# nitishsaDire/objectDetection_ssd

Measured on AMD Instinct MI355X. Metric: images/sec SSD300-VGG16 train step, higher is better.
Workload: dtype f32 (tensors, accumulators, loss, SGD; the Winograd-domain products of the layers with >= 256 reduction channels are formed from three EXACT bf16 limbs per f32 operand on the bf16 MFMA -- six limb products per f32 product, dropped terms <= 2^-26 -- measured no further from f64 than the f32 MFMA; SSD

## Files before the change

### include/ssd_gfx950.h

```cpp
#ifndef SSD_GFX950_H
#define SSD_GFX950_H

#include <stddef.h>
#include <stdint.h>

#ifdef __cplusplus
extern "C" {
#endif

#define SSD_ABI_VERSION 1

enum ssd_status {
    SSD_OK = 0,
    SSD_ERR_BAD_SHAPE = -1,
    SSD_ERR_WORKSPACE = -2,
    SSD_ERR_NULL = -3,
    SSD_ERR_LAUNCH = -4,
    SSD_ERR_ALIGN = -5
};

int ssd_abi_version(void);
const char* ssd_status_string(int status);

typedef struct ssd_conv_geom {
// ... 105 lines not shown
int ssd_wino4_dy_transform_pooled(const float* dpool, const unsigned char* argmax, const float* y_pooled, int Hp, int Wp, int ldy,
                                  const ssd_conv_geom* g, float* wgrad_planes, float* dgrad_planes_out, float* bias_partial, void* stream);
int ssd_conv3x3_wino_wgrad_planes_pooled(const float* planes, const float* dpool, const unsigned char* argmax, const float* y_pooled,
                                         int Hp, int Wp, int ldy, float* dw_oihw, float* dbias, const ssd_conv_geom* g,
                                         float* dgrad_planes_out, void* workspace, size_t workspace_bytes, void* stream);
int ssd_conv3x3_wino_fwd_keep_bits(const float* x, const float* U_fwd, const float* bias, float* y, int ldy, const ssd_conv_geom* g, int relu,
                                   float* planes_keep, uint64_t* relu_bits_out, void* workspace, size_t workspace_bytes, void* stream);
int ssd_conv3x3_wino_fwd_pool_bits(const float* x, const float* U_fwd, const float* bias, float* y_pooled, uint8_t* argmax,
                                   const ssd_conv_geom* g, int ceil_mode, float* planes_keep, uint64_t* relu_bits_out, void* workspace,
                                   size_t workspace_bytes, void* stream);
int ssd_conv3x3_wino_dgrad_bits(const float* dy, int ldy, const float* U_bwd, int Co_pad, float* dx, const uint64_t* relu_bits, int accumulate,
                                const ssd_conv_geom* g, void* workspace, size_t workspace_bytes, void* stream);
int ssd_conv3x3_wino_dgrad_planes_bits(const float* dy_planes, const float* U_bwd, int Co_pad, float* dx, const uint64_t* relu_bits,
                                       int accumulate, const ssd_conv_geom* g, void* workspace, size_t workspace_bytes, void* stream);
int ssd_conv3x3_wino_wgrad_planes(const float* planes, const float* dy, int ldy, float* dw_oihw, float* dbias, const ssd_conv_geom* g,
                                  float* dgrad_planes_out, void* workspace, size_t workspace_bytes, void* stream);
int ssd_conv3x3_wino_dgrad_planes(const float* dy_planes, const float* U_bwd, int Co_pad, float* dx, const float* relu_mask,
                                  int accumulate, const ssd_conv_geom* g, void* workspace, size_t workspace_bytes, void* stream);
int ssd_conv1_first_wino_fwd(const float* x_nchw, const float* w_rows, const float* bias, float* planes, uint64_t* relu_bits, int N, int H, int W,
                             void* stream);
int ssd_conv3x3_wino_fwd_from_planes(const float* planes, const float* U_fwd, const float* bias, float* y, int ldy, float* y_pooled, uint8_t* argmax,
                                     const ssd_conv_geom* g, int relu, int ceil_mode, void* workspace, size_t workspace_bytes, void* stream);
int ssd_wino_weights_adj(const float* w_oihw, float* U_adj, int Co, int Ci, int Co_pad, void* stream);
size_t ssd_wino4_adj_planes_floats(const ssd_conv_geom* g);
int ssd_conv3x3_wino_dgrad_adj_gemm(const float* y_planes, int ldy, const float* U_adj, float* md_planes, const ssd_conv_geom* g, void* stream);
int ssd_wino4_adj_output(const float* md_planes, float* dx, const float* relu_mask, const uint64_t* relu_bits, int accumulate,
                         const ssd_conv_geom* g, void* stream);
int ssd_wino4_adj_output_to_planes(const float* md_planes, const float* relu_mask, const uint64_t* relu_bits, const ssd_conv_geom* g,
                                   const ssd_conv_geom* g_below, float* y_planes, float* bias_partial, void* stream);
int ssd_tune_set_wino_bias_tail(int on);
int ssd_tune_set_wino_xform_blocks(int blocks);
int ssd_tune_set_wino_fused(int mode);
int ssd_gemm_planes_x3v2(const void* a3, const void* w3, float* out, int M, int K, int N, int n_rows, int nbatch, int dither, void* stream);
int ssd_tune_set_x3_big(int mode);
int ssd_tune_set_x3_mfma(int rows);
int ssd_tune_set_gemm_nt(int mode);
int ssd_wino_uses_x3(int mo, int K);
int ssd_tune_set_wino_x3(int on);
size_t ssd_gemm_x3_weights_bytes(int rows, int K, int nbatch);
int ssd_gemm_x3_split_weights(const float* w, void* w3, int rows, int K, int nbatch, void* stream);
int ssd_gemm_planes_x3(const float* a, const void* w3, float* out, int M, int K, int N, int n_rows, int nbatch, void* stream);
int ssd_conv1x1_fwd_x3(const float* x, const void* w3, const float* bias, float* y, int ldy, const ssd_conv_geom* g, int relu, void* stream);
int ssd_conv1x1_dgrad_x3(const float* dy, int ldy, const void* w3t, float* dx, const float* relu_mask, int accumulate, const ssd_conv_geom* g,
                         void* stream);
size_t ssd_conv1x1_wgrad_x3_workspace(const ssd_conv_geom* g, int ldy);
int ssd_conv1x1_wgrad_x3(const float* x, const float* dy, int ldy, float* dw, float* dbias, const ssd_conv_geom* g, void* workspace,
                         size_t workspace_bytes, void* stream);
int ssd_gemm_planes_f32(const float* a, const float* w, float* out, int M, int K, int N, int n_rows, int nbatch, void* stream);
int ssd_has_experimental(void);
int ssd_tune_set_wino_full(int mode);
int ssd_conv3x3_wino_uses_full(const ssd_conv_geom* g, int direction);
int ssd_tune_set_wino_fused_stagger(int cycles);
int ssd_tune_set_wino_fused_stamps(uint64_t* device_buffer);
int ssd_tune_set_wino_wgrad_tn(int on);
int ssd_prof_gemm_begin(void);
int ssd_prof_gemm_collect_kinds(float* ms_out, double* flops_out, int* kinds_out, int max);
int ssd_prof_gemm_collect(float* ms_out, double* flops_out, int max);
int ssd_tune_set_igemm(int tile, int nbuf);
int ssd_tune_set_igemm_stamps(uint64_t* device_buffer);
int ssd_tune_set_dgrad_parity(int on);
int ssd_tune_set_batched_units(int on);
int ssd_tune_set_igemm_lds_pad(int bytes);
int ssd_tune_set_wgrad(int bt, int nbuf, int blocks_per_cu);
int ssd_tune_set_wgrad_patch(int shape);

int ssd_im2col_first(const float* x_nchw, float* out, int N, int H, int W, void* stream);
int ssd_conv1_first_fwd(const float* x_nchw, const float* w_rows, const float* bias, float* y_nhwc, float* col_out, int N, int H, int W,
                        int relu, void* stream);
size_t ssd_conv1_first_wgrad_workspace(int N, int H, int W);
int ssd_conv1_first_wgrad(const float* x_nchw, const float* dy_nhwc, float* dw_rows, float* dbias, int N, int H, int W, void* workspace,
                          size_t workspace_bytes, void* stream);

int ssd_im2col_nchw3(const float* x_nchw, float* out, int N, int H, int W, int R, int S, int stride, int pad,
                     int Ho, int Wo, int Kpad, void* stream);
int ssd_conv2d_fwd_accum(const float* x, const float* w_ohwi, const float* bias, float* y_inout, int ldy,
                         const ssd_conv_geom* g, int relu, void* stream);
int ssd_conv2d_fwd_accum_bf16(const float* x, const float* w_ohwi, const float* bias, float* y_inout, int ldy,
                              const ssd_conv_geom* g, int relu, void* stream);
int ssd_channel_affine(const float* x, const float* scale, const float* shift, float* y, size_t M, int C, int relu,
                       void* stream);

int ssd_maxpool_fwd(const float* x, float* y, uint8_t* argmax, int N, int H, int W, int C,
                    int k, int stride, int pad, int Ho, int Wo, void* stream);
int ssd_maxpool_bwd(const float* dy, const uint8_t* argmax, float* dx, const float* relu_mask, int accumulate,
                    int N, int H, int W, int C, int k, int stride, int pad, int Ho, int Wo, void* stream);
int ssd_maxpool_bwd_gated(const float* dy, const uint8_t* argmax, const float* y, float* dx, int N, int H, int W, int C,
                          int k, int stride, int pad, int Ho, int Wo, void* stream);

int ssd_l2norm_fwd(const float* x, const float* gamma, float* y, int M, int C, void* stream);
size_t ssd_l2norm_bwd_workspace(int M, int C);
int ssd_l2norm_bwd(const float* x, const float* gamma, const float* dy, float* dx, float* dgamma,
                   int M, int C, void* workspace, size_t workspace_bytes, void* stream);

int ssd_heads_scatter(const float* packed, int ld, float* loc, float* conf, int N, int HW, int A,
                      int prior_off, int P, int n_classes, void* stream);
int ssd_heads_gather(const float* dloc, const float* dconf, float* packed, int ld, int N, int HW, int A,
                     int prior_off, int P, int n_classes, void* stream);

int ssd_tune_set_loss_form(int three_launch);
size_t ssd_multibox_loss_workspace(int bs, int P, int n_gt);
int ssd_multibox_loss(const float* loc, const float* conf, const float* gt_boxes, const float* gt_classes,
                      const int32_t* img_start, int bs, int n_gt, const float* priors_cxcywh,
                      const float* priors_xyxy, int P, int n_classes, float iou_threshold, int neg_pos_ratio,
                      int norm_mode, float* losses, int32_t* obj, int32_t* cls, float* dloc, float* dconf,
                      void* workspace, size_t workspace_bytes, void* stream);

// ... 80 lines not shown
```

### objectdetection_ssd_amd/_lib.py

```python
from __future__ import annotations

import ctypes as C
import os

PKG = os.path.dirname(os.path.abspath(__file__))
LIB_PATH = os.path.join(PKG, "libssd_gfx950.so")

SSD_ABI_VERSION = 1


class ConvGeom(C.Structure):
    _fields_ = [(n, C.c_int32) for n in ("N", "H", "W", "Ci", "Ho", "Wo", "Co", "R", "S", "stride", "pad", "dil")]


class ImageDesc(C.Structure):
    _fields_ = [("src_offset", C.c_int64)] + [(n, C.c_int32) for n in (
        "src_h", "src_w", "canvas_h", "canvas_w", "place_top", "place_left", "crop_top", "crop_left", "crop_h", "crop_w",
        "flip", "reserved")]


class WeightJob(C.Structure):
    _fields_ = [("w0", C.c_void_p), ("w1", C.c_void_p), ("out_fwd", C.c_void_p), ("out_bwd", C.c_void_p)] + [(n, C.c_int32) for n in (
        "co0", "co", "ci", "taps", "co_pad", "kind", "pad0", "pad1")]

# ... 76 lines not shown
    "ssd_conv3x3_halo_fwd_bf16": (_I, [_P, _P, _I, _P, _P, _I, _G, _I, _P]),
    "ssd_conv3x3_halo_dgrad_bf16": (_I, [_P, _I, _P, _I, _P, _P, _I, _G, _P]),
    "ssd_conv2d_wgrad_workspace": (_Z, [_G]),
    "ssd_conv2d_wgrad": (_I, [_P, _P, _I, _P, _P, _G, _P, _Z, _P]),
    "ssd_conv2d_igemm_tile": (_I, [_G, _I, C.POINTER(C.c_int), C.POINTER(C.c_int)]),
    "ssd_conv2d_wgrad_tile": (_I, [_G, C.POINTER(C.c_int), C.POINTER(C.c_int)]),
    "ssd_conv2d_wgrad_plan": (_I, [_G, _I, C.POINTER(C.c_int)]),
    "ssd_conv3x3_bf16_plan": (_I, [_I, _I, _I, _I, _I, C.POINTER(C.c_int)]),
    "ssd_conv3x3_halo_shape": (_I, [_G, _I, _I]),
    "ssd_conv2d_igemm_workspace": (_Z, [_G, _I]),
    "ssd_conv2d_fwd_ws": (_I, [_P, _P, _P, _P, _I, _G, _I, _P, _Z, _P]),
    "ssd_conv2d_dgrad_ws": (_I, [_P, _I, _P, _I, _P, _P, _I, _G, _P, _Z, _P]),
    "ssd_tune_set_igemm_splitk": (_I, [_I]),
    "ssd_wino_weights": (_I, [_P, _P, _P, _I, _I, _I, _I, _P]),
    "ssd_conv3x3_wino_workspace": (_Z, [_G, _I, _I]),
    "ssd_conv3x3_wino_fwd": (_I, [_P, _P, _P, _P, _I, _G, _I, _I, _P, _Z, _P]),
    "ssd_conv3x3_wino_fwd_pool": (_I, [_P, _P, _P, _P, _P, _G, _I, _P, _P, _Z, _P]),
    "ssd_conv3x3_wino_fwd_keep": (_I, [_P, _P, _P, _P, _I, _G, _I, _P, _P, _Z, _P]),
    "ssd_weight_job_blocks": (_I, [_P]),
    "ssd_weights_prepare": (_I, [_P, _P, _I, _I, _P]),
    "ssd_wino4_bias_partial_floats": (_Z, [_G, _I]),
    "ssd_wino4_dy_transform": (_I, [_P, _I, _G, _P, _P, _P, _P]),
    "ssd_wino_weights_adj": (_I, [_P, _P, _I, _I, _I, _P]),
    "ssd_conv1_first_wino_fwd": (_I, [_P, _P, _P, _P, _P, _I, _I, _I, _P]),
    "ssd_conv3x3_wino_fwd_from_planes": (_I, [_P, _P, _P, _P, _I, _P, _P, _G, _I, _I, _P, _Z, _P]),
    "ssd_wino4_adj_planes_floats": (_Z, [_G]),
    "ssd_conv3x3_wino_dgrad_adj_gemm": (_I, [_P, _I, _P, _P, _G, _P]),
    "ssd_wino4_adj_output": (_I, [_P, _P, _P, _P, _I, _G, _P]),
    "ssd_wino4_adj_output_to_planes": (_I, [_P, _P, _P, _G, _G, _P, _P, _P]),
    "ssd_wino4_dy_transform_pooled": (_I, [_P, _P, _P, _I, _I, _I, _G, _P, _P, _P, _P]),
    "ssd_conv3x3_wino_wgrad_planes_pooled": (_I, [_P, _P, _P, _P, _I, _I, _I, _P, _P, _G, _P, _P, _Z, _P]),
    "ssd_wino4_wgrad_gemm_workspace": (_Z, [_G, _I]),
    "ssd_wino4_wgrad_gemm": (_I, [_P, _P, _I, _P, _P, _P, _G, _P, _Z, _P]),
    "ssd_conv3x3_wino_fwd_keep_bits": (_I, [_P, _P, _P, _P, _I, _G, _I, _P, _P, _P, _Z, _P]),
    "ssd_conv3x3_wino_fwd_pool_bits": (_I, [_P, _P, _P, _P, _P, _G, _I, _P, _P, _P, _Z, _P]),
    "ssd_conv3x3_wino_dgrad_planes_bits": (_I, [_P, _P, _I, _P, _P, _I, _G, _P, _Z, _P]),
    "ssd_conv3x3_wino_wgrad_planes": (_I, [_P, _P, _I, _P, _P, _G, _P, _P, _Z, _P]),
    "ssd_conv3x3_wino_dgrad_planes": (_I, [_P, _P, _I, _P, _P, _I, _G, _P, _Z, _P]),
    "ssd_conv3x3_wino_dgrad": (_I, [_P, _I, _P, _I, _P, _P, _I, _G, _I, _P, _Z, _P]),
    "ssd_conv3x3_wino_wgrad_workspace": (_Z, [_G, _I, _I]),
    "ssd_conv3x3_wino_wgrad": (_I, [_P, _P, _I, _P, _P, _G, _I, _P, _Z, _P]),
    "ssd_tune_set_wino_wgrad_tn": (_I, [_I]),
    "ssd_tune_set_wino_fused": (_I, [_I]),
    "ssd_tune_set_gemm_nt": (_I, [_I]),
    "ssd_tune_set_wino_bias_tail": (_I, [_I]),
    "ssd_tune_set_batched_units": (_I, [_I]),
    "ssd_tune_set_dgrad_parity": (_I, [_I]),
    "ssd_tune_set_wino_full": (_I, [_I]),
    "ssd_conv3x3_wino_uses_full": (_I, [_G, _I]),
    "ssd_conv3x3_wino_dgrad_bits": (_I, [_P, _I, _P, _I, _P, _P, _I, _G, _P, _Z, _P]),
    "ssd_tune_set_wino_xform_blocks": (_I, [_I]),
    "ssd_tune_set_wino_fused_stamps": (_I, [_P]),
    "ssd_tune_set_wino_fused_stagger": (_I, [_I]),
    "ssd_prof_gemm_begin": (_I, []),
    "ssd_prof_gemm_collect": (_I, [_P, _P, _I]),
    "ssd_prof_gemm_collect_kinds": (_I, [_P, _P, _P, _I]),
    "ssd_tune_set_igemm": (_I, [_I, _I]),
    "ssd_tune_set_igemm_lds_pad": (_I, [_I]),
    "ssd_tune_set_igemm_stamps": (_I, [_P]),
    "ssd_tune_set_wgrad": (_I, [_I, _I, _I]),
    "ssd_tune_set_wgrad_patch": (_I, [_I]),
    "ssd_im2col_first": (_I, [_P, _P, _I, _I, _I, _P]),
    "ssd_conv1_first_fwd": (_I, [_P, _P, _P, _P, _P, _I, _I, _I, _I, _P]),
    "ssd_conv1_first_wgrad_workspace": (_Z, [_I, _I, _I]),
    "ssd_conv1_first_wgrad": (_I, [_P, _P, _P, _P, _I, _I, _I, _P, _Z, _P]),
    "ssd_maxpool_fwd": (_I, [_P, _P, _P, _I, _I, _I, _I, _I, _I, _I, _I, _I, _P]),
    "ssd_maxpool_bwd_gated": (_I, [_P, _P, _P, _P, _I, _I, _I, _I, _I, _I, _I, _I, _I, _P]),
    "ssd_maxpool_bwd": (_I, [_P, _P, _P, _P, _I, _I, _I, _I, _I, _I, _I, _I, _I, _I, _P]),
    "ssd_l2norm_fwd": (_I, [_P, _P, _P, _I, _I, _P]),
    "ssd_l2norm_bwd_workspace": (_Z, [_I, _I]),
    "ssd_l2norm_bwd": (_I, [_P, _P, _P, _P, _P, _I, _I, _P, _Z, _P]),
    "ssd_heads_scatter": (_I, [_P, _I, _P, _P, _I, _I, _I, _I, _I, _I, _P]),
    "ssd_heads_gather": (_I, [_P, _P, _P, _I, _I, _I, _I, _I, _I, _I, _P]),
    "ssd_multibox_loss_workspace": (_Z, [_I, _I, _I]),
    "ssd_multibox_loss": (_I, [_P, _P, _P, _P, _P, _I, _I, _P, _P, _I, _I, _F, _I, _I, _P, _P, _P, _P, _P, _P, _Z, _P]),
    "ssd_decode_nms_workspace": (_Z, [_I, _I]),
    "ssd_decode_nms": (_I, [_P, _P, _P, _I, _I, _F, _F, _I, _F, _F, _P, _P, _P, _P, _P, _P, _Z, _P]),
    "ssd_decode_nms_batch_workspace": (_Z, [_I, _I, _I]),
    "ssd_decode_nms_batch": (_I, [_P, _P, _P, _P, _I, _I, _I, _F, _F, _I, _P, _P, _P, _P, _P, _P, _Z, _P]),
    "ssd_sgd_momentum": (_I, [_P, _P, _P, _Z, _F, _F, _F, _P, _I, _P]),
    "ssd_bn_workspace": (_Z, [_Z, _I]),
    "ssd_bn_train_stats": (_I, [_P, _I, _Z, _I, _P, _P, _F, _F, _P, _P, _P, _P, _P, _P, _P, _P, _Z, _P]),
    "ssd_bn_apply": (_I, [_P, _I, _Z, _I, _P, _P, _P, _I, _P, _P, _I, _I, _F, _U64, _I, _I, _P, _I, _P]),
    "ssd_bn_train_bwd": (_I, [_P, _I, _P, _I, _Z, _I, _P, _P, _P, _I, _F, _U64, _I, _I, _I, _P, _P, _P, _I, _P, _I, _P, _Z, _P]),
    "ssd_dropout_mask": (_I, [_P, _Z, _F, _U64, _I, _P]),
}

_lib = None


def load() -> C.CDLL:
    global _lib
    if _lib is not None:
        return _lib
    import torch
    if not os.path.exists(LIB_PATH):
        from . import build as _build
        _build.build()
    try:
        lib = C.CDLL(LIB_PATH)
    except OSError as e:
        raise RuntimeError(f"cannot load {LIB_PATH}: {e}.  The gfx950 HIP extension is the only compute "
                           f"path of this package; build it with `python -m objectdetection_ssd_amd.build`.") from e
    for name, (res, args) in SIGNATURES.items():
        fn = getattr(lib, name)
        fn.restype = res
# ... 12 lines not shown
```

### objectdetection_ssd_amd/csrc/wino_fused.hip

```cpp
#include "common.h"

namespace {

__device__ constexpr float F4_AT[4][6] = {{1, 1, 1, 1, 1, 0}, {0, 1, -1, 2, -2, 0}, {0, 1, 1, 4, 4, 0}, {0, 1, -1, 8, -8, 1}};

struct FusedParams {
    const float* V;
    const float* U;
    size_t plane_v, plane_u;
    int tiles, K, Nrows, Nout;
    int groups, nblk_n;
    float* out; int ldo; int Cvalid;
    const float* bias; const float* mask; const unsigned long long* mask_bits; int relu, accumulate;
    int H, W, TH, TW;
    float* yp; uint8_t* am; int Ho, Wo;
    unsigned long long* stamps;
    int stagger;
};

constexpr int FG = 32, FN = 64, FK = 64;
#ifndef WF_NS
#define WF_NS 5
#define WF_PD 3
#endif
constexpr int NS = WF_NS, PD = WF_PD;
constexpr int STAGE_F = (FG + FN) * FK;
constexpr int LOADS = 3;
constexpr int YS_F = FG * 16 * FN;
constexpr int LDS_F = NS * STAGE_F > YS_F ? NS * STAGE_F : YS_F;
static_assert(NS - PD >= 2, "a slot is re-filled no earlier than two barriers after its last read");
static_assert(LDS_F * 4 <= 160 * 1024, "LDS");

typedef __attribute__((address_space(3))) void lds_void;

template <int N> __device__ __forceinline__ void wait_vmcnt() { asm volatile("s_waitcnt vmcnt(%0)" ::"n"(N) : "memory"); }

template <int KCN>
__global__ __launch_bounds__(512, 2) void wino4_gemm_out_kernel(const FusedParams p) {
    __shared__ __attribute__((aligned(16))) float lds[LDS_F];
    const int tid = threadIdx.x, lane = tid & 63;
    const int wave = __builtin_amdgcn_readfirstlane(tid >> 6);
    const int mb = wave >> 2, nbw = wave & 3;
    const int nblk = p.groups * p.nblk_n;
    const int lid = xcd_swizzle(blockIdx.x, nblk);
    const int grp = lid / p.nblk_n, nb = lid - grp * p.nblk_n;
    const int tile0 = grp * FG, n0 = nb * FN;
    constexpr int S = 36 * KCN;
    const bool stamp = p.stamps != nullptr && (blockIdx.x & 15) == 0 && tid == 0;
    unsigned long long ts[8] = {0, 0, 0, 0, 0, 0, 0, 0};
    if (stamp) ts[0] = __builtin_readcyclecounter();
    if (p.stagger > 0 && blockIdx.x < 256) {
        const long long want = (long long)((blockIdx.x >> 3) & 7) * p.stagger;
        const long long t0 = (long long)__builtin_readcyclecounter();
        while ((long long)__builtin_readcyclecounter() - t0 < want) __builtin_amdgcn_s_sleep(64);
    }

    const int lrow = lane >> 4, pc = lane & 15;
    unsigned src_off[LOADS];
    bool is_a[LOADS];
    int lds_off[LOADS];
#pragma unroll
    for (int i = 0; i < LOADS; ++i) {
        const int q = 3 * wave + i;
        is_a[i] = q < 8;
        const int row = is_a[i] ? 4 * q + lrow : 4 * (q - 8) + lrow;
        const int src_row = is_a[i] ? min(tile0 + row, p.tiles - 1) : min(n0 + row, p.Nrows - 1);
        src_off[i] = (unsigned)src_row * (unsigned)p.K + (unsigned)((pc ^ (row & 15)) * 4);
        lds_off[i] = q * 256;
    }
    auto issue = [&](int stage) {
        const int xi = stage / KCN, kc = stage % KCN, slot = stage % NS;
        const float* vsrc = p.V + (size_t)xi * p.plane_v + kc * FK;
        const float* usrc = p.U + (size_t)xi * p.plane_u + kc * FK;
        float* base = lds + slot * STAGE_F;
#pragma unroll
        for (int i = 0; i < LOADS; ++i)
            __builtin_amdgcn_global_load_lds((is_a[i] ? vsrc : usrc) + src_off[i], (lds_void*)(base + lds_off[i]), 16, 0, 0);
    };

    f32x4 acc[36];
#pragma unroll
    for (int xi = 0; xi < 36; ++xi) acc[xi] = f32x4{0.f, 0.f, 0.f, 0.f};

    const int r15 = lane & 15, kq = lane >> 4;
    const int a_rd = (mb * 16 + r15) * FK, b_rd = FG * FK + (nbw * 16 + r15) * FK;
    int sw[4];
#pragma unroll
    for (int j = 0; j < 4; ++j) sw[j] = ((4 * j + kq) ^ r15) * 4;

    struct Frag { f32x4 a[4], b[4]; };
    Frag F[2];
    auto load_frags = [&](Frag& f, int slot) {
        const float* st = lds + slot * STAGE_F;
#pragma unroll
        for (int j = 0; j < 4; ++j) {
            f.a[j] = *reinterpret_cast<const f32x4*>(st + a_rd + sw[j]);
            f.b[j] = *reinterpret_cast<const f32x4*>(st + b_rd + sw[j]);
        }
    };
    auto mma4 = [&](f32x4& c, const Frag& f, int j) {
#ifdef WF_NO_MFMA
        c += f.a[j] * f.b[j];
#else
#pragma unroll
        for (int e = 0; e < 4; ++e) c = __builtin_amdgcn_mfma_f32_16x16x4f32(f.a[j][e], f.b[j][e], c, 0, 0, 0);
#endif
    };

#pragma unroll
    for (int s = 0; s < PD; ++s)
        if (s < S) issue(s);
    wait_vmcnt<(PD < S ? PD - 1 : S - 1) * LOADS>();
    __builtin_amdgcn_s_barrier();
    asm volatile("" ::: "memory");
    load_frags(F[0], 0);
    if (stamp) ts[1] = __builtin_readcyclecounter();

#pragma clang loop unroll(full)
    for (int s = 0; s < S; ++s) {
        f32x4& c = acc[s / KCN];
        const Frag& cur = F[s & 1];
        Frag& nxt = F[(s & 1) ^ 1];
        mma4(c, cur, 0);
        __builtin_amdgcn_sched_barrier(0);
#ifndef WF_NO_LOAD
        if (s + PD < S) issue(s + PD);
#endif
        __builtin_amdgcn_sched_barrier(0);
        mma4(c, cur, 1);
        mma4(c, cur, 2);
        __builtin_amdgcn_sched_barrier(0);
        if (s + 1 < S) {
            const int issued = (s + PD + 1 < S ? s + PD + 1 : S);
            const int ahead = issued - s - 2;
            if (ahead >= 3) wait_vmcnt<3 * LOADS>();
            else if (ahead == 2) wait_vmcnt<2 * LOADS>();
            else if (ahead == 1) wait_vmcnt<LOADS>();
            else wait_vmcnt<0>();
            __builtin_amdgcn_s_barrier();
            asm volatile("" ::: "memory");
            load_frags(nxt, (s + 1) % NS);
        }
        __builtin_amdgcn_sched_barrier(0);
        mma4(c, cur, 3);
    }

    if (stamp) ts[2] = __builtin_readcyclecounter();
    float* ys = lds;
    const int C4 = p.Nout >> 2;
    __builtin_amdgcn_s_barrier();
#pragma unroll
    for (int r = 0; r < 4; ++r) {
        float t[4][6];
#pragma unroll
        for (int b = 0; b < 6; ++b) {
            const float m0 = acc[b][r], m1 = acc[6 + b][r], m2 = acc[12 + b][r], m3 = acc[18 + b][r], m4 = acc[24 + b][r], m5 = acc[30 + b][r];
            const float s1 = m1 + m2, d1 = m1 - m2, s2 = m3 + m4, d2 = m3 - m4;
            t[0][b] = m0 + s1 + s2;
            t[1][b] = d1 + 2.f * d2;
            t[2][b] = s1 + 4.f * s2;
            t[3][b] = d1 + 8.f * d2 + m5;
        }
        float* dst = ys + (size_t)((mb * 16 + 4 * kq + r) * 16) * FN + nbw * 16 + r15;
#pragma unroll
        for (int i = 0; i < 4; ++i) {
            const float s1 = t[i][1] + t[i][2], d1 = t[i][1] - t[i][2], s2 = t[i][3] + t[i][4], d2 = t[i][3] - t[i][4];
            dst[(i * 4 + 0) * FN] = t[i][0] + s1 + s2;
            dst[(i * 4 + 1) * FN] = d1 + 2.f * d2;
            dst[(i * 4 + 2) * FN] = s1 + 4.f * s2;
            dst[(i * 4 + 3) * FN] = d1 + 8.f * d2 + t[i][5];
        }
    }
    asm volatile("s_waitcnt lgkmcnt(0)" ::: "memory");
    __builtin_amdgcn_s_barrier();
    if (stamp) ts[3] = __builtin_readcyclecounter();
    {
        const int tl = tid >> 4, c4l = tid & 15;
        const int tile = tile0 + tl, c4 = (n0 >> 2) + c4l;
        if (tile < p.tiles && c4 < C4) {
            const int tw = tile % p.TW, th = (tile / p.TW) % p.TH, n = tile / (p.TW * p.TH);
            const float* src = ys + (size_t)(tl * 16) * FN + c4l * 4;
            f32x4 bv = {0.f, 0.f, 0.f, 0.f};
            if (p.bias != nullptr) {
#pragma unroll
                for (int e = 0; e < 4; ++e) bv[e] = c4 * 4 + e < p.Cvalid ? p.bias[c4 * 4 + e] : 0.f;
            }
            if (p.yp == nullptr) {
                const unsigned long long word = p.mask_bits != nullptr ? p.mask_bits[(size_t)tile * C4 + c4] : 0ull;
#pragma unroll
                for (int a = 0; a < 4; ++a) {
                    const int oh = 4 * th + a;
                    if (oh >= p.H) continue;
#pragma unroll
                    for (int b = 0; b < 4; ++b) {
                        const int ow = 4 * tw + b;
                        if (ow >= p.W) continue;
                        f32x4 v = *reinterpret_cast<const f32x4*>(src + (a * 4 + b) * FN) + bv;
                        const size_t idx = (((size_t)n * p.H + oh) * p.W + ow) * p.ldo + c4 * 4;
                        if (p.accumulate) v += *reinterpret_cast<const f32x4*>(p.out + idx);
                        if (p.relu) {
#pragma unroll
                            for (int e = 0; e < 4; ++e) v[e] = v[e] < 0.f ? 0.f : v[e];
                        }
                        if (p.mask_bits != nullptr) {
#pragma unroll
                            for (int e = 0; e < 4; ++e) v[e] = ((word >> ((a * 4 + b) * 4 + e)) & 1ull) ? v[e] : 0.f;
                        } else if (p.mask != nullptr) {
                            const f32x4 mk = *reinterpret_cast<const f32x4*>(p.mask + idx);
#pragma unroll
                            for (int e = 0; e < 4; ++e) v[e] = mk[e] > 0.f ? v[e] : 0.f;
                        }
                        *reinterpret_cast<f32x4*>(p.out + idx) = v;
                    }
                }
            } else {
#pragma unroll
                for (int pa = 0; pa < 2; ++pa) {
                    const int oh = 2 * th + pa;
                    if (oh >= p.Ho) continue;
#pragma unroll
                    for (int pb = 0; pb < 2; ++pb) {
                        const int ow = 2 * tw + pb;
                        if (ow >= p.Wo) continue;
                        f32x4 best = {-INFINITY, -INFINITY, -INFINITY, -INFINITY};
                        int bi[4] = {0, 0, 0, 0};
                        bool first = true;
#pragma unroll
                        for (int r = 0; r < 2; ++r) {
                            if (2 * oh + r >= p.H) continue;
#pragma unroll
                            for (int q = 0; q < 2; ++q) {
                                if (2 * ow + q >= p.W) continue;
                                f32x4 v = *reinterpret_cast<const f32x4*>(src + ((2 * pa + r) * 4 + 2 * pb + q) * FN) + bv;
#pragma unroll
                                for (int e = 0; e < 4; ++e) {
                                    v[e] = v[e] < 0.f ? 0.f : v[e];
                                    if (first || v[e] > best[e] || v[e] != v[e]) {
                                        best[e] = v[e];
                                        bi[e] = r * 2 + q;
                                    }
                                }
                                first = false;
                            }
                        }
                        const size_t o = (((size_t)n * p.Ho + oh) * p.Wo + ow) * C4 + c4;
                        *reinterpret_cast<f32x4*>(p.yp + o * 4) = best;
                        if (p.am != nullptr)
                            *reinterpret_cast<uint32_t*>(p.am + o * 4) =
                                (uint32_t)bi[0] | ((uint32_t)bi[1] << 8) | ((uint32_t)bi[2] << 16) | ((uint32_t)bi[3] << 24);
                    }
                }
            }
        }
    }
    if (stamp) {
        ts[4] = __builtin_readcyclecounter();
        asm volatile("s_waitcnt vmcnt(0)" ::: "memory");
        unsigned long long* o = p.stamps + (size_t)(blockIdx.x >> 4) * 8;
        for (int i = 0; i < 5; ++i) o[i] = ts[i];
        o[5] = __builtin_readcyclecounter();
    }
}

}
int ssd_internal_prof_open(double flops, int kind, hipStream_t st);
void ssd_internal_prof_close(int slot, hipStream_t st);
namespace {
unsigned long long* g_fused_stamps = nullptr;
int g_fused_stagger = -1;
}

extern "C" int ssd_tune_set_wino_fused_stagger(int cycles) {
    g_fused_stagger = cycles;
    return SSD_OK;
}
extern "C" int ssd_tune_set_wino_fused_stamps(uint64_t* device_buffer) {
    g_fused_stamps = reinterpret_cast<unsigned long long*>(device_buffer);
    return SSD_OK;
}

__attribute__((visibility("hidden"))) int ssd_internal_wino4_gemm_out(const float* V, const float* U, int tiles, int K, int Nrows, int Nout,
                                                                       float* out, int ldo, int Cvalid, const float* bias, const float* mask,
                                                                       const unsigned long long* mask_bits, int relu, int accumulate, int H, int W,
                                                                       int TH, int TW, float* yp, uint8_t* am, int Ho, int Wo, hipStream_t st) {
    if ((K != 64 && K != 128 && K != 256) || tiles <= 0 || Nout <= 0 || Nout % 4 != 0 || Nrows <= 0) return SSD_ERR_BAD_SHAPE;
    if ((size_t)tiles * K >= (1ull << 32) || (size_t)Nrows * K >= (1ull << 32)) return SSD_ERR_BAD_SHAPE;
    FusedParams p;
    p.V = V; p.U = U;
    p.plane_v = (size_t)tiles * K; p.plane_u = (size_t)Nrows * K;
    p.tiles = tiles; p.K = K; p.Nrows = Nrows; p.Nout = Nout;
    p.groups = ssd_cdiv(tiles, FG); p.nblk_n = ssd_cdiv(Nout, FN);
    p.out = out; p.ldo = ldo; p.Cvalid = Cvalid; p.bias = bias; p.mask = mask; p.mask_bits = mask_bits; p.relu = relu; p.accumulate = accumulate;
    p.H = H; p.W = W; p.TH = TH; p.TW = TW;
    p.yp = yp; p.am = am; p.Ho = Ho; p.Wo = Wo;
    p.stamps = g_fused_stamps;
    p.stagger = g_fused_stagger < 0 ? 0 : g_fused_stagger;
    const long long nblk = (long long)p.groups * p.nblk_n;
    if (nblk >= (1ll << 31)) return SSD_ERR_BAD_SHAPE;
    const int slot = ssd_internal_prof_open(2.0 * 36 * tiles * (double)K * (double)(p.nblk_n * FN), 1, st);
    switch (K / FK) {
        case 1: hipLaunchKernelGGL(wino4_gemm_out_kernel<1>, dim3((unsigned)nblk), dim3(512), 0, st, p); break;
        case 2: hipLaunchKernelGGL(wino4_gemm_out_kernel<2>, dim3((unsigned)nblk), dim3(512), 0, st, p); break;
        case 4: hipLaunchKernelGGL(wino4_gemm_out_kernel<4>, dim3((unsigned)nblk), dim3(512), 0, st, p); break;
        default: return SSD_ERR_BAD_SHAPE;
    }
    ssd_internal_prof_close(slot, st);
    SSD_CHECK_LAUNCH();
    return SSD_OK;
}

namespace {

__device__ constexpr float F4_BT[6][6] = {{4, 0, -5, 0, 1, 0}, {0, -4, -4, 1, 1, 0}, {0, 4, -4, -1, 1, 0},
                                          {0, -2, -1, 2, 1, 0}, {0, 2, -1, -2, 1, 0}, {0, 4, 0, -5, 0, 1}};

struct FullParams {
    const float* x;
    unsigned x_bytes;
    const float* U;
    size_t plane_u;
    int tiles, K, Nrows, Nout, groups, nblk_n;
    float* out; int ldo; int Cvalid;
    const float* bias; const float* mask; const unsigned long long* mask_bits; int relu, accumulate;
    int H, W, TH, TW;
    float* yp; uint8_t* am; int Ho, Wo;
    float* V_keep;
    unsigned long long* bits_out;
    unsigned long long* stamps;
};

#ifdef SSD_EXPERIMENTAL
constexpr int GT = 32;
constexpr int KH = 32;
constexpr int VS_F = 36 * GT * KH;
typedef float f32x2 __attribute__((ext_vector_type(2)));

template <int KP>
__global__ __launch_bounds__(512, 2) void wino4_full_kernel(const FullParams p) {
    __shared__ __attribute__((aligned(16))) float lds[VS_F];
    const int tid = threadIdx.x, lane = tid & 63;
    const int wave = __builtin_amdgcn_readfirstlane(tid >> 6);
    const int nbw = wave & 3, mb = wave >> 2;
    const int nblk = p.groups * p.nblk_n;
    const int lid = xcd_swizzle(blockIdx.x, nblk);
    const int grp = lid / p.nblk_n, nb = lid - grp * p.nblk_n;
    const int tile0 = grp * GT, n0 = nb * FN;
    const int r15 = lane & 15, kq = lane >> 4;
    const bool stamp = p.stamps != nullptr && (blockIdx.x & 15) == 0 && tid == 0;
    unsigned long long ts[8] = {0, 0, 0, 0, 0, 0, 0, 0};
    if (stamp) ts[0] = __builtin_readcyclecounter();

    f32x4 acc[36];
#pragma unroll
    for (int i = 0; i < 36; ++i) acc[i] = f32x4{0.f, 0.f, 0.f, 0.f};

    const int brow = min(n0 + nbw * 16 + r15, p.Nrows - 1);
// ... 263 lines not shown
```

Measured before the change: 1612.

## Make fused Winograd GEMM kernel persistent with grid capped at CU count

The fused Winograd GEMM+output-transform kernel now loops over work tiles with a grid-stride loop, and by default launches at most one block per CU instead of one block per tile. The epilogue also reads the whole 16-pixel tile out of LDS into registers and then hits a barrier before the global stores, so the next iteration can safely reuse the LDS. The aim is to cut block launch and prologue overhead and even out the tail. The risk is lower occupancy: launch bounds allow two blocks per CU but the grid caps at one per CU. Each block also loses the overlap between one tile's epilogue and the next tile's loads, and the extra barrier plus register pressure could hurt.

```diff
diff --git a/include/ssd_gfx950.h b/include/ssd_gfx950.h
--- a/include/ssd_gfx950.h
+++ b/include/ssd_gfx950.h
@@ -181,6 +181,8 @@
 int ssd_conv3x3_wino_uses_full(const ssd_conv_geom* g, int direction);
 int ssd_tune_set_wino_fused_stagger(int cycles);
 int ssd_tune_set_wino_fused_stamps(uint64_t* device_buffer);
+int ssd_tune_set_wino_fused_persistent(int mode);
+int ssd_tune_set_wino_fused_grid(int blocks);
 int ssd_tune_set_wino_wgrad_tn(int on);
 int ssd_prof_gemm_begin(void);
 int ssd_prof_gemm_collect_kinds(float* ms_out, double* flops_out, int* kinds_out, int max);
diff --git a/objectdetection_ssd_amd/_lib.py b/objectdetection_ssd_amd/_lib.py
--- a/objectdetection_ssd_amd/_lib.py
+++ b/objectdetection_ssd_amd/_lib.py
@@ -152,6 +152,8 @@
     "ssd_tune_set_wino_xform_blocks": (_I, [_I]),
     "ssd_tune_set_wino_fused_stamps": (_I, [_P]),
     "ssd_tune_set_wino_fused_stagger": (_I, [_I]),
+    "ssd_tune_set_wino_fused_persistent": (_I, [_I]),
+    "ssd_tune_set_wino_fused_grid": (_I, [_I]),
     "ssd_prof_gemm_begin": (_I, []),
     "ssd_prof_gemm_collect": (_I, [_P, _P, _I]),
     "ssd_prof_gemm_collect_kinds": (_I, [_P, _P, _P, _I]),
diff --git a/objectdetection_ssd_amd/csrc/wino_fused.hip b/objectdetection_ssd_amd/csrc/wino_fused.hip
--- a/objectdetection_ssd_amd/csrc/wino_fused.hip
+++ b/objectdetection_ssd_amd/csrc/wino_fused.hip
@@ -42,13 +42,7 @@
     const int wave = __builtin_amdgcn_readfirstlane(tid >> 6);
     const int mb = wave >> 2, nbw = wave & 3;
     const int nblk = p.groups * p.nblk_n;
-    const int lid = xcd_swizzle(blockIdx.x, nblk);
-    const int grp = lid / p.nblk_n, nb = lid - grp * p.nblk_n;
-    const int tile0 = grp * FG, n0 = nb * FN;
     constexpr int S = 36 * KCN;
-    const bool stamp = p.stamps != nullptr && (blockIdx.x & 15) == 0 && tid == 0;
-    unsigned long long ts[8] = {0, 0, 0, 0, 0, 0, 0, 0};
-    if (stamp) ts[0] = __builtin_readcyclecounter();
     if (p.stagger > 0 && blockIdx.x < 256) {
         const long long want = (long long)((blockIdx.x >> 3) & 7) * p.stagger;
         const long long t0 = (long long)__builtin_readcyclecounter();
@@ -58,30 +52,26 @@
     const int lrow = lane >> 4, pc = lane & 15;
     unsigned src_off[LOADS];
     bool is_a[LOADS];
-    int lds_off[LOADS];
+    int lds_off[LOADS], prow[LOADS];
 #pragma unroll
     for (int i = 0; i < LOADS; ++i) {
         const int q = 3 * wave + i;
         is_a[i] = q < 8;
-        const int row = is_a[i] ? 4 * q + lrow : 4 * (q - 8) + lrow;
-        const int src_row = is_a[i] ? min(tile0 + row, p.tiles - 1) : min(n0 + row, p.Nrows - 1);
-        src_off[i] = (unsigned)src_row * (unsigned)p.K + (unsigned)((pc ^ (row & 15)) * 4);
+        prow[i] = is_a[i] ? 4 * q + lrow : 4 * (q - 8) + lrow;
         lds_off[i] = q * 256;
     }
+    const float *Vb = p.V, *Ub = p.U;
+    size_t plane_v = p.plane_v, plane_u = p.plane_u;
     auto issue = [&](int stage) {
         const int xi = stage / KCN, kc = stage % KCN, slot = stage % NS;
-        const float* vsrc = p.V + (size_t)xi * p.plane_v + kc * FK;
-        const float* usrc = p.U + (size_t)xi * p.plane_u + kc * FK;
+        const float* vsrc = Vb + (size_t)xi * plane_v + kc * FK;
+        const float* usrc = Ub + (size_t)xi * plane_u + kc * FK;
         float* base = lds + slot * STAGE_F;
 #pragma unroll
         for (int i = 0; i < LOADS; ++i)
             __builtin_amdgcn_global_load_lds((is_a[i] ? vsrc : usrc) + src_off[i], (lds_void*)(base + lds_off[i]), 16, 0, 0);
     };
 
-    f32x4 acc[36];
-#pragma unroll
-    for (int xi = 0; xi < 36; ++xi) acc[xi] = f32x4{0.f, 0.f, 0.f, 0.f};
-
     const int r15 = lane & 15, kq = lane >> 4;
     const int a_rd = (mb * 16 + r15) * FK, b_rd = FG * FK + (nbw * 16 + r15) * FK;
     int sw[4];
@@ -89,7 +79,6 @@
     for (int j = 0; j < 4; ++j) sw[j] = ((4 * j + kq) ^ r15) * 4;
 
     struct Frag { f32x4 a[4], b[4]; };
-    Frag F[2];
     auto load_frags = [&](Frag& f, int slot) {
         const float* st = lds + slot * STAGE_F;
 #pragma unroll
@@ -107,158 +96,186 @@
 #endif
     };
 
-#pragma unroll
-    for (int s = 0; s < PD; ++s)
-        if (s < S) issue(s);
-    wait_vmcnt<(PD < S ? PD - 1 : S - 1) * LOADS>();
-    __builtin_amdgcn_s_barrier();
-    asm volatile("" ::: "memory");
-    load_frags(F[0], 0);
-    if (stamp) ts[1] = __builtin_readcyclecounter();
+    for (int lid0 = blockIdx.x; lid0 < nblk; lid0 += gridDim.x) {
+        const int lid = xcd_swizzle(lid0, nblk);
+        const int grp = lid / p.nblk_n, nb = lid - grp * p.nblk_n;
+        const int tile0 = grp * FG, n0 = nb * FN;
+        const bool stamp = p.stamps != nullptr && (lid0 & 15) == 0 && tid == 0;
+        unsigned long long ts[8] = {0, 0, 0, 0, 0, 0, 0, 0};
+        if (stamp) ts[0] = __builtin_readcyclecounter();
+        asm volatile("" : "+s"(Vb), "+s"(Ub), "+s"(plane_v), "+s"(plane_u));
+#pragma unroll
+        for (int i = 0; i < LOADS; ++i) {
+            const int src_row = is_a[i] ? min(tile0 + prow[i], p.tiles - 1) : min(n0 + prow[i], p.Nrows - 1);
+            src_off[i] = (unsigned)src_row * (unsigned)p.K + (unsigned)((pc ^ (prow[i] & 15)) * 4);
+        }
+
+        f32x4 acc[36];
+#pragma unroll
+        for (int xi = 0; xi < 36; ++xi) acc[xi] = f32x4{0.f, 0.f, 0.f, 0.f};
+        Frag F[2];
+
+#pragma unroll
+        for (int s = 0; s < PD; ++s)
+            if (s < S) issue(s);
+        wait_vmcnt<(PD < S ? PD - 1 : S - 1) * LOADS>();
+        __builtin_amdgcn_s_barrier();
+        asm volatile("" ::: "memory");
+        load_frags(F[0], 0);
+        if (stamp) ts[1] = __builtin_readcyclecounter();
 
 #pragma clang loop unroll(full)
-    for (int s = 0; s < S; ++s) {
-        f32x4& c = acc[s / KCN];
-        const Frag& cur = F[s & 1];
-        Frag& nxt = F[(s & 1) ^ 1];
-        mma4(c, cur, 0);
-        __builtin_amdgcn_sched_barrier(0);
+        for (int s = 0; s < S; ++s) {
+            f32x4& c = acc[s / KCN];
+            const Frag& cur = F[s & 1];
+            Frag& nxt = F[(s & 1) ^ 1];
+            mma4(c, cur, 0);
+            __builtin_amdgcn_sched_barrier(0);
 #ifndef WF_NO_LOAD
-        if (s + PD < S) issue(s + PD);
+            if (s + PD < S) issue(s + PD);
 #endif
-        __builtin_amdgcn_sched_barrier(0);
-        mma4(c, cur, 1);
-        mma4(c, cur, 2);
-        __builtin_amdgcn_sched_barrier(0);
-        if (s + 1 < S) {
-            const int issued = (s + PD + 1 < S ? s + PD + 1 : S);
-            const int ahead = issued - s - 2;
-            if (ahead >= 3) wait_vmcnt<3 * LOADS>();
-            else if (ahead == 2) wait_vmcnt<2 * LOADS>();
-            else if (ahead == 1) wait_vmcnt<LOADS>();
-            else wait_vmcnt<0>();
+            __builtin_amdgcn_sched_barrier(0);
+            mma4(c, cur, 1);
+            mma4(c, cur, 2);
+            __builtin_amdgcn_sched_barrier(0);
+            if (s + 1 < S) {
+                const int issued = (s + PD + 1 < S ? s + PD + 1 : S);
+                const int ahead = issued - s - 2;
+                if (ahead >= 3) wait_vmcnt<3 * LOADS>();
+                else if (ahead == 2) wait_vmcnt<2 * LOADS>();
+                else if (ahead == 1) wait_vmcnt<LOADS>();
+                else wait_vmcnt<0>();
+                __builtin_amdgcn_s_barrier();
+                asm volatile("" ::: "memory");
+                load_frags(nxt, (s + 1) % NS);
+            }
+            __builtin_amdgcn_sched_barrier(0);
+            mma4(c, cur, 3);
+        }
+
+        if (stamp) ts[2] = __builtin_readcyclecounter();
+        float* ys = lds;
+        const int C4 = p.Nout >> 2;
+        __builtin_amdgcn_s_barrier();
+#pragma unroll
+        for (int r = 0; r < 4; ++r) {
+            float t[4][6];
+#pragma unroll
+            for (int b = 0; b < 6; ++b) {
+                const float m0 = acc[b][r], m1 = acc[6 + b][r], m2 = acc[12 + b][r], m3 = acc[18 + b][r], m4 = acc[24 + b][r], m5 = acc[30 + b][r];
+                const float s1 = m1 + m2, d1 = m1 - m2, s2 = m3 + m4, d2 = m3 - m4;
+                t[0][b] = m0 + s1 + s2;
+                t[1][b] = d1 + 2.f * d2;
+                t[2][b] = s1 + 4.f * s2;
+                t[3][b] = d1 + 8.f * d2 + m5;
+            }
+            float* dst = ys + (size_t)((mb * 16 + 4 * kq + r) * 16) * FN + nbw * 16 + r15;
+#pragma unroll
+            for (int i = 0; i < 4; ++i) {
+                const float s1 = t[i][1] + t[i][2], d1 = t[i][1] - t[i][2], s2 = t[i][3] + t[i][4], d2 = t[i][3] - t[i][4];
+                dst[(i * 4 + 0) * FN] = t[i][0] + s1 + s2;
+                dst[(i * 4 + 1) * FN] = d1 + 2.f * d2;
+                dst[(i * 4 + 2) * FN] = s1 + 4.f * s2;
+                dst[(i * 4 + 3) * FN] = d1 + 8.f * d2 + t[i][5];
+            }
+        }
+        asm volatile("s_waitcnt lgkmcnt(0)" ::: "memory");
+        __builtin_amdgcn_s_barrier();
+        asm volatile("" ::: "memory");
+        if (stamp) ts[3] = __builtin_readcyclecounter();
+        {
+            const int tl = tid >> 4, c4l = tid & 15;
+            const int tile = tile0 + tl, c4 = (n0 >> 2) + c4l;
+            f32x4 px[16];
+#pragma unroll
+            for (int i = 0; i < 16; ++i) px[i] = *reinterpret_cast<const f32x4*>(ys + (size_t)(tl * 16 + i) * FN + c4l * 4);
+            asm volatile("s_waitcnt lgkmcnt(0)" ::: "memory");
             __builtin_amdgcn_s_barrier();
             asm volatile("" ::: "memory");
-            load_frags(nxt, (s + 1) % NS);
-        }
-        __builtin_amdgcn_sched_barrier(0);
-        mma4(c, cur, 3);
-    }
-
-    if (stamp) ts[2] = __builtin_readcyclecounter();
-    float* ys = lds;
-    const int C4 = p.Nout >> 2;
-    __builtin_amdgcn_s_barrier();
-#pragma unroll
-    for (int r = 0; r < 4; ++r) {
-        float t[4][6];
-#pragma unroll
-        for (int b = 0; b < 6; ++b) {
-            const float m0 = acc[b][r], m1 = acc[6 + b][r], m2 = acc[12 + b][r], m3 = acc[18 + b][r], m4 = acc[24 + b][r], m5 = acc[30 + b][r];
-            const float s1 = m1 + m2, d1 = m1 - m2, s2 = m3 + m4, d2 = m3 - m4;
-            t[0][b] = m0 + s1 + s2;
-            t[1][b] = d1 + 2.f * d2;
-            t[2][b] = s1 + 4.f * s2;
-            t[3][b] = d1 + 8.f * d2 + m5;
-        }
-        float* dst = ys + (size_t)((mb * 16 + 4 * kq + r) * 16) * FN + nbw * 16 + r15;
-#pragma unroll
-        for (int i = 0; i < 4; ++i) {
-            const float s1 = t[i][1] + t[i][2], d1 = t[i][1] - t[i][2], s2 = t[i][3] + t[i][4], d2 = t[i][3] - t[i][4];
-            dst[(i * 4 + 0) * FN] = t[i][0] + s1 + s2;
-            dst[(i * 4 + 1) * FN] = d1 + 2.f * d2;
-            dst[(i * 4 + 2) * FN] = s1 + 4.f * s2;
-            dst[(i * 4 + 3) * FN] = d1 + 8.f * d2 + t[i][5];
-        }
-    }
-    asm volatile("s_waitcnt lgkmcnt(0)" ::: "memory");
-    __builtin_amdgcn_s_barrier();
-    if (stamp) ts[3] = __builtin_readcyclecounter();
-    {
-        const int tl = tid >> 4, c4l = tid & 15;
-        const int tile = tile0 + tl, c4 = (n0 >> 2) + c4l;
-        if (tile < p.tiles && c4 < C4) {
-            const int tw = tile % p.TW, th = (tile / p.TW) % p.TH, n = tile / (p.TW * p.TH);
-            const float* src = ys + (size_t)(tl * 16) * FN + c4l * 4;
-            f32x4 bv = {0.f, 0.f, 0.f, 0.f};
-            if (p.bias != nullptr) {
-#pragma unroll
-                for (int e = 0; e < 4; ++e) bv[e] = c4 * 4 + e < p.Cvalid ? p.bias[c4 * 4 + e] : 0.f;
-            }
-            if (p.yp == nullptr) {
-                const unsigned long long word = p.mask_bits != nullptr ? p.mask_bits[(size_t)tile * C4 + c4] : 0ull;
-#pragma unroll
-                for (int a = 0; a < 4; ++a) {
-                    const int oh = 4 * th + a;
-                    if (oh >= p.H) continue;
-#pragma unroll
-                    for (int b = 0; b < 4; ++b) {
-                        const int ow = 4 * tw + b;
-                        if (ow >= p.W) continue;
-                        f32x4 v = *reinterpret_cast<const f32x4*>(src + (a * 4 + b) * FN) + bv;
-                        const size_t idx = (((size_t)n * p.H + oh) * p.W + ow) * p.ldo + c4 * 4;
-                        if (p.accumulate) v += *reinterpret_cast<const f32x4*>(p.out + idx);
-                        if (p.relu) {
-#pragma unroll
-                            for (int e = 0; e < 4; ++e) v[e] = v[e] < 0.f ? 0.f : v[e];
+            if (tile < p.tiles && c4 < C4) {
+                const int tw = tile % p.TW, th = (tile / p.TW) % p.TH, n = tile / (p.TW * p.TH);
+                f32x4 bv = {0.f, 0.f, 0.f, 0.f};
+                if (p.bias != nullptr) {
+#pragma unroll
+                    for (int e = 0; e < 4; ++e) bv[e] = c4 * 4 + e < p.Cvalid ? p.bias[c4 * 4 + e] : 0.f;
+                }
+                asm volatile("" ::"v"(bv));
+                if (p.yp == nullptr) {
+                    const unsigned long long word = p.mask_bits != nullptr ? p.mask_bits[(size_t)tile * C4 + c4] : 0ull;
+                    asm volatile("" ::"v"(word));
+#pragma unroll
+                    for (int a = 0; a < 4; ++a) {
+                        const int oh = 4 * th + a;
+                        if (oh >= p.H) continue;
+#pragma unroll
+                        for (int b = 0; b < 4; ++b) {
+                            const int ow = 4 * tw + b;
+                            if (ow >= p.W) continue;
+                            f32x4 v = px[a * 4 + b] + bv;
+                            const size_t idx = (((size_t)n * p.H + oh) * p.W + ow) * p.ldo + c4 * 4;
+                            if (p.accumulate) v += *reinterpret_cast<const f32x4*>(p.out + idx);
+                            if (p.relu) {
+#pragma unroll
+                                for (int e = 0; e < 4; ++e) v[e] = v[e] < 0.f ? 0.f : v[e];
+                            }
+                            if (p.mask_bits != nullptr) {
+#pragma unroll
+                                for (int e = 0; e < 4; ++e) v[e] = ((word >> ((a * 4 + b) * 4 + e)) & 1ull) ? v[e] : 0.f;
+                            } else if (p.mask != nullptr) {
+                                const f32x4 mk = *reinterpret_cast<const f32x4*>(p.mask + idx);
+#pragma unroll
+                                for (int e = 0; e < 4; ++e) v[e] = mk[e] > 0.f ? v[e] : 0.f;
+                            }
+                            *reinterpret_cast<f32x4*>(p.out + idx) = v;
                         }
-                        if (p.mask_bits != nullptr) {
-#pragma unroll
-                            for (int e = 0; e < 4; ++e) v[e] = ((word >> ((a * 4 + b) * 4 + e)) & 1ull) ? v[e] : 0.f;
-                        } else if (p.mask != nullptr) {
-                            const f32x4 mk = *reinterpret_cast<const f32x4*>(p.mask + idx);
-#pragma unroll
-                            for (int e = 0; e < 4; ++e) v[e] = mk[e] > 0.f ? v[e] : 0.f;
+                    }
+                } else {
+#pragma unroll
+                    for (int pa = 0; pa < 2; ++pa) {
+                        const int oh = 2 * th + pa;
+                        if (oh >= p.Ho) continue;
+#pragma unroll
+                        for (int pb = 0; pb < 2; ++pb) {
+                            const int ow = 2 * tw + pb;
+                            if (ow >= p.Wo) continue;
+                            f32x4 best = {-INFINITY, -INFINITY, -INFINITY, -INFINITY};
+                            int bi[4] = {0, 0, 0, 0};
+                            bool first = true;
+#pragma unroll
+                            for (int r = 0; r < 2; ++r) {
+                                if (2 * oh + r >= p.H) continue;
+#pragma unroll
+                                for (int q = 0; q < 2; ++q) {
+                                    if (2 * ow + q >= p.W) continue;
+                                    f32x4 v = px[(2 * pa + r) * 4 + 2 * pb + q] + bv;
+#pragma unroll
+                                    for (int e = 0; e < 4; ++e) {
+                                        v[e] = v[e] < 0.f ? 0.f : v[e];
+                                        if (first || v[e] > best[e] || v[e] != v[e]) {
+                                            best[e] = v[e];
+                                            bi[e] = r * 2 + q;
+                                        }
+                                    }
+                                    first = false;
+                                }
+                            }
+                            const size_t o = (((size_t)n * p.Ho + oh) * p.Wo + ow) * C4 + c4;
+                            *reinterpret_cast<f32x4*>(p.yp + o * 4) = best;
+                            if (p.am != nullptr)
+                                *reinterpret_cast<uint32_t*>(p.am + o * 4) =
+                                    (uint32_t)bi[0] | ((uint32_t)bi[1] << 8) | ((uint32_t)bi[2] << 16) | ((uint32_t)bi[3] << 24);
                         }
-                        *reinterpret_cast<f32x4*>(p.out + idx) = v;
                     }
                 }
-            } else {
-#pragma unroll
-                for (int pa = 0; pa < 2; ++pa) {
-                    const int oh = 2 * th + pa;
-                    if (oh >= p.Ho) continue;
-#pragma unroll
-                    for (int pb = 0; pb < 2; ++pb) {
-                        const int ow = 2 * tw + pb;
-                        if (ow >= p.Wo) continue;
-                        f32x4 best = {-INFINITY, -INFINITY, -INFINITY, -INFINITY};
-                        int bi[4] = {0, 0, 0, 0};
-                        bool first = true;
-#pragma unroll
-                        for (int r = 0; r < 2; ++r) {
-                            if (2 * oh + r >= p.H) continue;
-#pragma unroll
-                            for (int q = 0; q < 2; ++q) {
-                                if (2 * ow + q >= p.W) continue;
-                                f32x4 v = *reinterpret_cast<const f32x4*>(src + ((2 * pa + r) * 4 + 2 * pb + q) * FN) + bv;
-#pragma unroll
-                                for (int e = 0; e < 4; ++e) {
-                                    v[e] = v[e] < 0.f ? 0.f : v[e];
-                                    if (first || v[e] > best[e] || v[e] != v[e]) {
-                                        best[e] = v[e];
-                                        bi[e] = r * 2 + q;
-                                    }
-                                }
-                                first = false;
-                            }
-                        }
-                        const size_t o = (((size_t)n * p.Ho + oh) * p.Wo + ow) * C4 + c4;
-                        *reinterpret_cast<f32x4*>(p.yp + o * 4) = best;
-                        if (p.am != nullptr)
-                            *reinterpret_cast<uint32_t*>(p.am + o * 4) =
-                                (uint32_t)bi[0] | ((uint32_t)bi[1] << 8) | ((uint32_t)bi[2] << 16) | ((uint32_t)bi[3] << 24);
-                    }
-                }
-            }
-        }
-    }
-    if (stamp) {
-        ts[4] = __builtin_readcyclecounter();
-        asm volatile("s_waitcnt vmcnt(0)" ::: "memory");
-        unsigned long long* o = p.stamps + (size_t)(blockIdx.x >> 4) * 8;
-        for (int i = 0; i < 5; ++i) o[i] = ts[i];
-        o[5] = __builtin_readcyclecounter();
+            }
+        }
+        if (stamp) {
+            ts[4] = __builtin_readcyclecounter();
+            asm volatile("s_waitcnt vmcnt(0)" ::: "memory");
+            unsigned long long* o = p.stamps + (size_t)(lid0 >> 4) * 8;
+            for (int i = 0; i < 5; ++i) o[i] = ts[i];
+            o[5] = __builtin_readcyclecounter();
+        }
     }
 }
 
@@ -268,6 +285,20 @@
 namespace {
 unsigned long long* g_fused_stamps = nullptr;
 int g_fused_stagger = -1;
+int g_fused_persistent = -1;
+int g_fused_grid = 0;
+
+int fused_cu_count() {
+    static std::atomic<int> cus[64];
+    int dev = 0;
+    if (hipGetDevice(&dev) != hipSuccess) return 0;
+    int n = cus[dev & 63].load(std::memory_order_relaxed);
+    if (n == 0) {
+        if (hipDeviceGetAttribute(&n, hipDeviceAttributeMultiprocessorCount, dev) != hipSuccess || n <= 0) return 0;
+        cus[dev & 63].store(n, std::memory_order_relaxed);
+    }
+    return n;
+}
 }
 
 extern "C" int ssd_tune_set_wino_fused_stagger(int cycles) {
@@ -276,6 +307,16 @@
 }
 extern "C" int ssd_tune_set_wino_fused_stamps(uint64_t* device_buffer) {
     g_fused_stamps = reinterpret_cast<unsigned long long*>(device_buffer);
+    return SSD_OK;
+}
+extern "C" int ssd_tune_set_wino_fused_persistent(int mode) {
+    if (mode < -1 || mode > 1) return SSD_ERR_BAD_SHAPE;
+    g_fused_persistent = mode;
+    return SSD_OK;
+}
+extern "C" int ssd_tune_set_wino_fused_grid(int blocks) {
+    if (blocks < 0) return SSD_ERR_BAD_SHAPE;
+    g_fused_grid = blocks;
     return SSD_OK;
 }
 
@@ -298,10 +339,17 @@
     const long long nblk = (long long)p.groups * p.nblk_n;
     if (nblk >= (1ll << 31)) return SSD_ERR_BAD_SHAPE;
     const int slot = ssd_internal_prof_open(2.0 * 36 * tiles * (double)K * (double)(p.nblk_n * FN), 1, st);
+    long long grid = nblk;
+    if (g_fused_persistent != 0) {
+        const int cus = fused_cu_count();
+        if (cus <= 0) return SSD_ERR_LAUNCH;
+        const long long cap = g_fused_grid > 0 && g_fused_grid < cus ? g_fused_grid : cus;
+        if (grid > cap) grid = cap;
+    }
     switch (K / FK) {
-        case 1: hipLaunchKernelGGL(wino4_gemm_out_kernel<1>, dim3((unsigned)nblk), dim3(512), 0, st, p); break;
-        case 2: hipLaunchKernelGGL(wino4_gemm_out_kernel<2>, dim3((unsigned)nblk), dim3(512), 0, st, p); break;
-        case 4: hipLaunchKernelGGL(wino4_gemm_out_kernel<4>, dim3((unsigned)nblk), dim3(512), 0, st, p); break;
+        case 1: hipLaunchKernelGGL(wino4_gemm_out_kernel<1>, dim3((unsigned)grid), dim3(512), 0, st, p); break;
+        case 2: hipLaunchKernelGGL(wino4_gemm_out_kernel<2>, dim3((unsigned)grid), dim3(512), 0, st, p); break;
+        case 4: hipLaunchKernelGGL(wino4_gemm_out_kernel<4>, dim3((unsigned)grid), dim3(512), 0, st, p); break;
         default: return SSD_ERR_BAD_SHAPE;
     }
     ssd_internal_prof_close(slot, st);
```

Result: no change. 1619 (median of 6 runs) (+0.4%).
